# panshengyi/MemVul

Measured on AMD Instinct MI355X. Metric: issue-reports/sec at seq_len=256 (BERT-base issue encoder + 124-anchor memory match), higher is better.
Workload: dtype fp16 + fp8 (MV_F16X8: fp16 MFMA sweep + one OCP-e4m3 MFMA correction sweep per GEMM, fp32 accumulate); 1 GPU; BASELINE.json configs[1]: 1xMI355X-per-rank, bert-base-uncased geometry (12 layers), seq_len=256, batch=256, 124-anchor CWE memory, compute dtype MV_F16X8; seeded random-init weights, synthetic token ids resident in HBM; compute=precise, global_batch=256, seq_len=256, anchors=124, parallelism=dp1 (corpus shards, one all-gather of (score,label) stats), stats_transport=none (one rank)

## Files before the change

### memvul_amd/csrc/gemm_pp.h

```cpp
#pragma once
#include "common.h"
#include <type_traits>
#include "gemm.h"

enum { PP_QK = 1, PP_GELU = 3, PP_RESLN3 = 8 };
constexpr int PP_F = 4;

#define PP_LDS_A 0
#define PP_LDS_B 65536
#define PP_LDS_BIAS 131072
#define PP_LDS_SCR (PP_LDS_BIAS + MV_INTER * 4)
#define PP_LDS_BYTES (PP_LDS_SCR + 8 * 2048)
#define PP_LDS_BIAS_T PP_LDS_BIAS
#define PP_LDS_STATS (PP_LDS_BIAS + 2048)
#define PP_LDS_SCR_RAW (PP_LDS_STATS + 2 * 6144)
#define PP_LDS_RSTD (PP_LDS_SCR_RAW + 8 * 2048)
#define PP_LDS_BYTES_RAW (PP_LDS_RSTD + 2048)

__device__ __forceinline__ uint32_t pack_h2(float a, float b) {
  const half2_t h = {(half_t)a, (half_t)b};
  return __builtin_bit_cast(uint32_t, h);
}

__device__ __forceinline__ void pin_f32x4(float& a, float& b, float& c, float& d) {
#if defined(__HIP_DEVICE_COMPILE__)
  asm("" : "+v"(a), "+v"(b), "+v"(c), "+v"(d));
#endif
}

__device__ __forceinline__ uint32_t f2u(float x) { return __float_as_uint(x); }
__device__ __forceinline__ float u2f(uint32_t x) { return __uint_as_float(x); }
typedef uint32_t u32x2 __attribute__((ext_vector_type(2)));
typedef uint32_t u32x4 __attribute__((ext_vector_type(4)));
typedef int intx4 __attribute__((ext_vector_type(4)));
typedef int intx8 __attribute__((ext_vector_type(8)));

__device__ __forceinline__ void scr_f16x2(uint32_t w0, uint32_t w1, uint32_t w2, uint32_t w3, const u32x2 (&da)[4],
                                          const u32x2 (&db)[4], uint32_t r, u32x4 (&o)[4]) {
#if defined(__HIP_DEVICE_COMPILE__)
  asm volatile(
      "ds_write_b64 %4, %8\n\tds_write_b64 %5, %9\n\tds_write_b64 %6, %10\n\tds_write_b64 %7, %11\n\t"
      "ds_read_b128 %0, %16\n\tds_read_b128 %1, %16 offset:1024\n\t"
      "ds_write_b64 %4, %12\n\tds_write_b64 %5, %13\n\tds_write_b64 %6, %14\n\tds_write_b64 %7, %15\n\t"
      "ds_read_b128 %2, %16\n\tds_read_b128 %3, %16 offset:1024\n\ts_waitcnt lgkmcnt(0)"
      : "=&v"(o[0]), "=&v"(o[1]), "=&v"(o[2]), "=&v"(o[3])
      : "v"(w0), "v"(w1), "v"(w2), "v"(w3), "v"(da[0]), "v"(da[1]), "v"(da[2]), "v"(da[3]), "v"(db[0]), "v"(db[1]),
        "v"(db[2]), "v"(db[3]), "v"(r)
      : "memory");
#endif
}
__device__ __forceinline__ void scr_f8x2(uint32_t w0, uint32_t w1, uint32_t w2, uint32_t w3, const uint32_t (&da)[8],
                                           const uint32_t (&db)[8], uint32_t r, u32x4 (&o)[4]) {
#if defined(__HIP_DEVICE_COMPILE__)
  asm volatile(
      "ds_write_b32 %4, %8\n\tds_write_b32 %5, %9\n\tds_write_b32 %6, %10\n\tds_write_b32 %7, %11\n\t"
      "ds_write_b32 %4, %12 offset:1024\n\tds_write_b32 %5, %13 offset:1024\n\tds_write_b32 %6, %14 offset:1024\n\tds_write_b32 %7, %15 offset:1024\n\t"
      "ds_read_b128 %0, %24\n\tds_read_b128 %1, %24 offset:1024\n\t"
      "ds_write_b32 %4, %16\n\tds_write_b32 %5, %17\n\tds_write_b32 %6, %18\n\tds_write_b32 %7, %19\n\t"
      "ds_write_b32 %4, %20 offset:1024\n\tds_write_b32 %5, %21 offset:1024\n\tds_write_b32 %6, %22 offset:1024\n\tds_write_b32 %7, %23 offset:1024\n\t"
      "ds_read_b128 %2, %24\n\tds_read_b128 %3, %24 offset:1024\n\ts_waitcnt lgkmcnt(0)"
      : "=&v"(o[0]), "=&v"(o[1]), "=&v"(o[2]), "=&v"(o[3])
      : "v"(w0), "v"(w1), "v"(w2), "v"(w3), "v"(da[0]), "v"(da[1]), "v"(da[2]), "v"(da[3]), "v"(da[4]), "v"(da[5]), "v"(da[6]),
        "v"(da[7]), "v"(db[0]), "v"(db[1]), "v"(db[2]), "v"(db[3]), "v"(db[4]), "v"(db[5]), "v"(db[6]), "v"(db[7]), "v"(r)
      : "memory");
#endif
}
__device__ __forceinline__ void scr_f8x1(uint32_t w0, uint32_t w1, uint32_t w2, uint32_t w3, const uint32_t (&da)[8], uint32_t r, u32x4 (&o)[4]) {
#if defined(__HIP_DEVICE_COMPILE__)
  asm volatile(
      "ds_write_b32 %2, %6\n\tds_write_b32 %3, %7\n\tds_write_b32 %4, %8\n\tds_write_b32 %5, %9\n\t"
      "ds_write_b32 %2, %10 offset:1024\n\tds_write_b32 %3, %11 offset:1024\n\tds_write_b32 %4, %12 offset:1024\n\tds_write_b32 %5, %13 offset:1024\n\t"
      "ds_read_b128 %0, %14\n\tds_read_b128 %1, %14 offset:1024\n\ts_waitcnt lgkmcnt(0)"
      : "=&v"(o[0]), "=&v"(o[1])
      : "v"(w0), "v"(w1), "v"(w2), "v"(w3), "v"(da[0]), "v"(da[1]), "v"(da[2]), "v"(da[3]), "v"(da[4]), "v"(da[5]), "v"(da[6]), "v"(da[7]), "v"(r)
      : "memory");
#endif
}
__device__ __forceinline__ void scr_f16x2_t(uint32_t t0, uint32_t t1, const u32x2 (&da)[4], const u32x2 (&db)[4], uint32_t r, u32x4 (&o)[4]) {
#if defined(__HIP_DEVICE_COMPILE__)
  const uint32_t a00 = da[0][0], a01 = da[0][1], a10 = da[1][0], a11 = da[1][1], a20 = da[2][0], a21 = da[2][1], a30 = da[3][0],
                 a31 = da[3][1];
  const uint32_t b00 = db[0][0], b01 = db[0][1], b10 = db[1][0], b11 = db[1][1], b20 = db[2][0], b21 = db[2][1], b30 = db[3][0],
                 b31 = db[3][1];
#define MV_T16(A, LO, HI, OFF)                                                                            \
  "ds_write_b16 " A ", " LO " offset:" #OFF "+0\n\tds_write_b16_d16_hi " A ", " LO " offset:" #OFF "+64\n\t" \
  "ds_write_b16 " A ", " HI " offset:" #OFF "+128\n\tds_write_b16_d16_hi " A ", " HI " offset:" #OFF "+192\n\t"
  asm volatile(
      MV_T16("%4", "%6", "%7", 0) MV_T16("%4", "%8", "%9", 1024) MV_T16("%5", "%10", "%11", 0) MV_T16("%5", "%12", "%13", 1024)
      "ds_read_b128 %0, %22\n\tds_read_b128 %1, %22 offset:1024\n\t"
      MV_T16("%4", "%14", "%15", 0) MV_T16("%4", "%16", "%17", 1024) MV_T16("%5", "%18", "%19", 0) MV_T16("%5", "%20", "%21", 1024)
      "ds_read_b128 %2, %22\n\tds_read_b128 %3, %22 offset:1024\n\ts_waitcnt lgkmcnt(0)"
      : "=&v"(o[0]), "=&v"(o[1]), "=&v"(o[2]), "=&v"(o[3])
      : "v"(t0), "v"(t1), "v"(a00), "v"(a01), "v"(a10), "v"(a11), "v"(a20), "v"(a21), "v"(a30), "v"(a31), "v"(b00), "v"(b01),
        "v"(b10), "v"(b11), "v"(b20), "v"(b21), "v"(b30), "v"(b31), "v"(r)
      : "memory");
#undef MV_T16
#endif
}
__device__ __forceinline__ void scr_f16_rev2(uint32_t wc, const u32x4& a0, const u32x4& a1, const u32x4& b0, const u32x4& b1, uint32_t r0,
                                             uint32_t r1, uint32_t r2, uint32_t r3, u32x2 (&oa)[4], u32x2 (&ob)[4]) {
#if defined(__HIP_DEVICE_COMPILE__)
  asm volatile(
      "ds_write_b128 %8, %9\n\tds_write_b128 %8, %10 offset:1024\n\t"
      "ds_read_b64 %0, %13\n\tds_read_b64 %1, %14\n\tds_read_b64 %2, %15\n\tds_read_b64 %3, %16\n\t"
      "ds_write_b128 %8, %11\n\tds_write_b128 %8, %12 offset:1024\n\t"
      "ds_read_b64 %4, %13\n\tds_read_b64 %5, %14\n\tds_read_b64 %6, %15\n\tds_read_b64 %7, %16\n\ts_waitcnt lgkmcnt(0)"
      : "=&v"(oa[0]), "=&v"(oa[1]), "=&v"(oa[2]), "=&v"(oa[3]), "=&v"(ob[0]), "=&v"(ob[1]), "=&v"(ob[2]), "=&v"(ob[3])
      : "v"(wc), "v"(a0), "v"(a1), "v"(b0), "v"(b1), "v"(r0), "v"(r1), "v"(r2), "v"(r3)
      : "memory");
  __builtin_amdgcn_sched_barrier(0);
#endif
}


__device__ __forceinline__ void lds_read_bgb1(uint32_t addr, float4& bi, float4& ga, float4& be) {
#if defined(__HIP_DEVICE_COMPILE__)
  asm volatile("ds_read_b128 %0, %3\n\tds_read_b128 %1, %3 offset:3072\n\tds_read_b128 %2, %3 offset:6144\n\ts_waitcnt lgkmcnt(0)"
               : "=&v"(bi), "=&v"(ga), "=&v"(be)
               : "v"(addr)
               : "memory");
  __builtin_amdgcn_sched_barrier(0);
#endif
}

__device__ __forceinline__ int sload_i32(const int* p) {
  int v = 0;
#if defined(__HIP_DEVICE_COMPILE__)
  asm volatile("s_load_dword %0, %1, 0x0\n\ts_waitcnt lgkmcnt(0)" : "=s"(v) : "s"(p) : "memory");
#endif
  return v;
}

__device__ __forceinline__ void raster_pp(const GemmArgs& a, int L, int G, int tm_count, int tn_count, int& tile_m, int& tile_n) {
  if (a.raster_mode == 1) {
    const int ngroups = tn_count / a.GN;
    const int w = L / G, r = L - w * G;
    const int b = w / ngroups, g = w - b * ngroups;
    const int p = b * G + r;
    tile_m = p / a.GN;
    tile_n = g * a.GN + (p - tile_m * a.GN);
  } else {
    raster(L, tm_count, tn_count, a.GN, tile_m, tile_n);
  }
}

template <int EPI, int RAW = 0, int X8 = 0>
__global__ __launch_bounds__(512, 2) void gemm_pp_kernel(GemmArgs a) {
  static_assert(EPI == PP_QK || EPI == PP_GELU || EPI == PP_RESLN3, "kernel kinds of the encoder layer");
  static_assert(RAW == (EPI != PP_RESLN3), "PP_QK / PP_GELU consume the raw stream (virtual LayerNorm), PP_RESLN3 produces it");
  constexpr bool IS_RES = (EPI == PP_RESLN3);
  static_assert(X8 == 0 || X8 == 1, "X8 = 1: MV_F16X8 (the fp8 correction sweep)");
  constexpr int WAITN = 2 * PP_F;
  constexpr int LDS_SCR = RAW ? PP_LDS_SCR_RAW : PP_LDS_SCR;
  extern __shared__ __attribute__((aligned(16))) char smem[];
  const int tid = threadIdx.x;
  const int lane = tid & 63;
  const int hi = lane >> 5, l31 = lane & 31;
  const int wave = __builtin_amdgcn_readfirstlane(tid >> 6);
  const int wr = wave >> 2, wc = wave & 3;
  const int K = a.K, nk0 = K >> 6;
  constexpr int nseg = X8 ? 2 : 1;
  auto short_tile = [&](int tm) -> bool { return a.tile_both && sload_i32(a.tile_both + tm) != 0; };
  auto both_terms = [&](int tm, int tn) -> bool {
    if (a.x8_terms == 1) return short_tile(tm);
    if (a.x8_terms != 3) return true;
    const int which = (tn * 256 + a.col0) / MV_HIDDEN;
    return (a.x8_aside_mask >> which) & 1;
  };
  int i_nk8 = X8 ? nk0 : 0;
  size_t i_off8 = 0;
  const int tm_count = a.M >> 8, tn_count = a.N >> 8;
  const int ntiles = tm_count * tn_count;
  const int G = gridDim.x;
  const int bslot = xcd_remap(blockIdx.x, G);

  if constexpr (!RAW) {
    float* lb = (float*)(smem + PP_LDS_BIAS);
    for (int n = tid; n < a.N; n += 512) lb[n] = a.bias ? a.bias[n] : 0.f;
    for (int n = tid; n < MV_HIDDEN; n += 512) {
      lb[MV_HIDDEN + n] = a.lng[n];
      lb[2 * MV_HIDDEN + n] = a.lnb[n];
    }
  }

  uint32_t offA[2], offB[2];
#pragma unroll
  for (int j = 0; j < 2; ++j) {
    const int rho = (2 * wave + j) * 8 + (lane >> 3);
    const int c = (lane & 7) ^ ((rho >> 1) & 7);
    const int rowA = (rho >> 6) * 128 + (rho & 63);
    const int rowB = (rho >> 5) * 64 + (rho & 31);
    offA[j] = (uint32_t)(rowA * K + c * 8) * 2u;
    offB[j] = (uint32_t)(rowB * K + c * 8) * 2u;
  }
  int i_it = 0, i_kt = 0, i_seg = 0;
  const char* iA = (const char*)a.A;
  const char* iW = (const char*)a.W;
  size_t tA = 0, tW = 0;
  auto set_issue_seg = [&]() {
    iA = (i_seg ? (const char*)a.A8 + i_off8 : (const char*)a.A) + tA;
    iW = (i_seg ? (const char*)a.W8 + i_off8 : (const char*)a.W) + tW;
  };
  auto set_issue_tile = [&](int it) {
    const int L = it * G + bslot;
    if (L < ntiles) {
      int tm, tn;
      raster_pp(a, L, G, tm_count, tn_count, tm, tn);
      if constexpr (X8) {
        tA = (size_t)tm * 256 * K * 2;
        tW = (size_t)tn * 256 * K * 2;
        const bool both = both_terms(tm, tn);
        i_nk8 = both ? nk0 : nk0 >> 1;
        i_off8 = both ? 0 : (size_t)K;
      } else {
        iA = (const char*)a.A + (size_t)tm * 256 * K * 2;
        iW = (const char*)a.W + (size_t)tn * 256 * K * 2;
      }
    }
    if constexpr (X8) set_issue_seg();
  };
  set_issue_tile(0);
  auto issue = [&](auto kindc, auto parc) {
    constexpr int kind = decltype(kindc)::value;
    constexpr int par = decltype(parc)::value;
    const char* src;
    char* dst;
    if constexpr (kind < 2) {
      src = iA + (size_t)(kind * 64) * K * 2 + i_kt * 128;
      dst = smem + PP_LDS_A + par * 32768 + kind * 16384 + wave * 2048;
      glds16((const half_t*)(src + offA[0]), dst);
      glds16((const half_t*)(src + offA[1]), dst + 1024);
    } else {
      src = iW + (size_t)((kind - 2) * 32) * K * 2 + i_kt * 128;
      dst = smem + PP_LDS_B + par * 32768 + (kind - 2) * 16384 + wave * 2048;
      glds16((const half_t*)(src + offB[0]), dst);
      glds16((const half_t*)(src + offB[1]), dst + 1024);
    }
    if constexpr (kind == 1) {
      if (++i_kt == ((X8 && i_seg) ? i_nk8 : nk0)) {
        i_kt = 0;
        if constexpr (X8) {
          if (++i_seg == nseg) {
            i_seg = 0;
            set_issue_tile(++i_it);
          } else {
            set_issue_seg();
          }
        } else {
          set_issue_tile(++i_it);
        }
      }
    }
  };
  auto issue_psi = [&](auto psic) {
    constexpr int psi = decltype(psic)::value;
    constexpr int q = psi & 3;
    constexpr int kind = (q == 0) ? 2 : (q == 1) ? 0 : (q == 2) ? 3 : 1;
    issue(std::integral_constant<int, kind>{}, std::integral_constant<int, (psi >> 2) & 1>{});
  };

  const int m16 = lane & 15, q4 = lane >> 4;
  int rdA[2], rdB[2];
#pragma unroll
  for (int kk = 0; kk < 2; ++kk) {
    const int o = m16 * 128 + (((4 * kk + q4) ^ ((m16 >> 1) & 7)) << 4);
    rdA[kk] = PP_LDS_A + wr * 8192 + o;
    rdB[kk] = PP_LDS_B + wc * 4096 + o;
  }
  half8_t Xf[X8 ? 1 : 4][X8 ? 1 : 2], Wx[X8 ? 1 : 2][X8 ? 1 : 2], Wy[X8 ? 1 : 2][X8 ? 1 : 2];
  intx8 Xp[X8 ? 4 : 1], Wxp[X8 ? 2 : 1], Wyp[X8 ? 2 : 1];
  auto ld16 = [&](int off) -> intx4 { return *(const intx4*)(smem + off); };
  auto read_a = [&](int par, int asub) {
#pragma unroll
    for (int t4 = 0; t4 < 4; ++t4) {
      const int o = par * 32768 + asub * 16384 + t4 * 2048;
      if constexpr (X8) {
        Xp[t4] = __builtin_shufflevector(ld16(rdA[0] + o), ld16(rdA[1] + o), 0, 1, 2, 3, 4, 5, 6, 7);
      } else {
#pragma unroll
        for (int kk = 0; kk < 2; ++kk) Xf[t4][kk] = *(const half8_t*)(smem + rdA[kk] + o);
      }
    }
  };
  auto read_b = [&](half8_t (&Wf)[X8 ? 1 : 2][X8 ? 1 : 2], intx8 (&Wp)[X8 ? 2 : 1], int par, int bsub) {
#pragma unroll
    for (int c2 = 0; c2 < 2; ++c2) {
      const int o = par * 32768 + bsub * 16384 + c2 * 2048;
      if constexpr (X8) {
        Wp[c2] = __builtin_shufflevector(ld16(rdB[0] + o), ld16(rdB[1] + o), 0, 1, 2, 3, 4, 5, 6, 7);
      } else {
#pragma unroll
        for (int kk = 0; kk < 2; ++kk) Wf[c2][kk] = *(const half8_t*)(smem + rdB[kk] + o);
      }
    }
  };

  floatx4 acc[8][4];
  auto park_residual = [&](int i, int mw0, int nw0) {
    const int crow = lane >> 2, cchunk = lane & 3;
    bool sp_c = false;
    size_t sp_off = 0;
    if constexpr (X8) {
      if ((i & 1) == 0) {
        const int row0 = mw0 + 32 * i, b = row0 / a.S;
        sp_c = row0 < a.Mreal && b * a.S == row0 && crow < 2;
        sp_off = (size_t)(2 * b + crow) * MV_HIDDEN;
      }
    }
#pragma unroll
    for (int j = 0; j < 2; ++j)
#pragma unroll
      for (int pl = 0; pl < 2; ++pl)
#pragma unroll
        for (int x = 0; x < 2; ++x) {
          const size_t row = (size_t)(mw0 + i * 32 + x * 16 + crow);
          if constexpr (X8) {
            if (pl == 1) {
              float4 t;
              if ((i & 1) == 0 && x == 0 && sp_c) {
                t = *(const float4*)(a.sp_lo_out + sp_off + nw0 + j * 32 + 8 * cchunk);
              } else {
                const float2 u = *(const float2*)(a.out8 + row * (2 * MV_HIDDEN) + nw0 + j * 32 + 8 * cchunk);
                t.x = u.x; t.y = u.y; t.z = 0.f; t.w = 0.f;
              }
              acc[2 * i + 1][2 * j + x][0] = t.x; acc[2 * i + 1][2 * j + x][1] = t.y; acc[2 * i + 1][2 * j + x][2] = t.z; acc[2 * i + 1][2 * j + x][3] = t.w;
              continue;
            }
          }
          const float4 t = *(const float4*)((pl ? a.out16b : a.out16) + row * MV_HIDDEN + nw0 + j * 32 + 8 * cchunk);
          acc[2 * i + pl][2 * j + x][0] = t.x; acc[2 * i + pl][2 * j + x][1] = t.y;
          acc[2 * i + pl][2 * j + x][2] = t.z; acc[2 * i + pl][2 * j + x][3] = t.w;
        }
  };
  auto mma_quadrant = [&](auto asubc, auto bc, auto f8c, const half8_t (&Wf)[X8 ? 1 : 2][X8 ? 1 : 2], const intx8 (&Wp)[X8 ? 2 : 1]) {
    constexpr int asub = decltype(asubc)::value;
    constexpr int b = decltype(bc)::value;
    if constexpr (X8) {
      if constexpr (decltype(f8c)::value) {
#pragma unroll
        for (int c2 = 0; c2 < 2; ++c2)
#pragma unroll
          for (int t4 = 0; t4 < 4; ++t4)
            acc[asub * 4 + t4][b * 2 + c2] = __builtin_amdgcn_mfma_scale_f32_16x16x128_f8f6f4(Wp[c2], Xp[t4], acc[asub * 4 + t4][b * 2 + c2], 0, 0, 0,
                                                                                            a.x8_scale, 0, 0x7f7f7f7f);
      } else {
#pragma unroll
        for (int kk = 0; kk < 2; ++kk)
#pragma unroll
          for (int c2 = 0; c2 < 2; ++c2) {
            const intx4 w4 = kk ? __builtin_shufflevector(Wp[c2], Wp[c2], 4, 5, 6, 7) : __builtin_shufflevector(Wp[c2], Wp[c2], 0, 1, 2, 3);
#pragma unroll
            for (int t4 = 0; t4 < 4; ++t4) {
              const intx4 x4 = kk ? __builtin_shufflevector(Xp[t4], Xp[t4], 4, 5, 6, 7) : __builtin_shufflevector(Xp[t4], Xp[t4], 0, 1, 2, 3);
              acc[asub * 4 + t4][b * 2 + c2] = __builtin_amdgcn_mfma_f32_16x16x32_f16(__builtin_bit_cast(half8_t, w4), __builtin_bit_cast(half8_t, x4),
                                                                                   acc[asub * 4 + t4][b * 2 + c2], 0, 0, 0);
            }
          }
      }
    } else {
#pragma unroll
      for (int kk = 0; kk < 2; ++kk)
#pragma unroll
        for (int c2 = 0; c2 < 2; ++c2)
#pragma unroll
          for (int t4 = 0; t4 < 4; ++t4)
            acc[asub * 4 + t4][b * 2 + c2] = __builtin_amdgcn_mfma_f32_16x16x32_f16(Wf[c2][kk], Xf[t4][kk], acc[asub * 4 + t4][b * 2 + c2], 0, 0, 0);
    }
  };

  auto read_set = [&](auto sc) {
    constexpr int s = decltype(sc)::value & 7;
    constexpr int P = s & 3, par = s >> 2;
    if constexpr (P == 0) { read_a(par, 0); read_b(Wx, Wxp, par, 0); }
    if constexpr (P == 1) read_b(Wy, Wyp, par, 1);
    if constexpr (P == 2) read_a(par, 1);
  };
  auto mma_set = [&](auto sc, auto f8c) {
    constexpr int P = decltype(sc)::value & 3;
    if constexpr (P == 0) mma_quadrant(std::integral_constant<int, 0>{}, std::integral_constant<int, 0>{}, f8c, Wx, Wxp);
    if constexpr (P == 1) mma_quadrant(std::integral_constant<int, 0>{}, std::integral_constant<int, 1>{}, f8c, Wy, Wyp);
    if constexpr (P == 2) mma_quadrant(std::integral_constant<int, 1>{}, std::integral_constant<int, 1>{}, f8c, Wy, Wyp);
    if constexpr (P == 3) mma_quadrant(std::integral_constant<int, 1>{}, std::integral_constant<int, 0>{}, f8c, Wx, Wxp);
  };
  auto interval = [&](auto sc, auto grpc, auto f8c, bool last_of_tile = false) {
    constexpr int s = decltype(sc)::value;
    constexpr int grp = decltype(grpc)::value;
    if constexpr (grp == 0) {
      __builtin_amdgcn_s_setprio(1);
      mma_set(sc, f8c);
      __builtin_amdgcn_s_setprio(0);
      __builtin_amdgcn_sched_barrier(0);
      if (!(s == 7 && last_of_tile)) read_set(std::integral_constant<int, (s + 1) & 7>{});
      issue_psi(std::integral_constant<int, (s + 3 + PP_F) & 7>{});
    } else {
      read_set(sc);
      issue_psi(std::integral_constant<int, (s + 3 + PP_F) & 7>{});
      __builtin_amdgcn_sched_barrier(0);
      mma_set(sc, f8c);
    }
    if constexpr (X8) {
#if defined(__HIP_DEVICE_COMPILE__)
      constexpr int P = s & 3, a0 = (P >= 2) ? 4 : 0, bq = (P == 1 || P == 2) ? 2 : 0;
      asm volatile("" : "+v"(acc[a0][bq]), "+v"(acc[a0 + 1][bq]), "+v"(acc[a0 + 2][bq]), "+v"(acc[a0 + 3][bq]), "+v"(acc[a0][bq + 1]),
                   "+v"(acc[a0 + 1][bq + 1]), "+v"(acc[a0 + 2][bq + 1]), "+v"(acc[a0 + 3][bq + 1]));
#endif
    }
    asm volatile("s_waitcnt vmcnt(%0)" ::"n"(WAITN) : "memory");
    __builtin_amdgcn_sched_barrier(0);
    __builtin_amdgcn_s_barrier();
    __builtin_amdgcn_sched_barrier(0);
  };

  auto issue_stats = [&](int itn, int tm, int tn) {
    if (itn * G + bslot < ntiles && wave < 4) {
#pragma unroll
      for (int pc = 0; pc < 2; ++pc) {
        const int piece = 2 * wave + pc;
        if (piece < 6) {
          const char* src = (const char*)a.lnstats + (size_t)tm * 6144 + piece * 1024 + lane * 16;
          glds16((const half_t*)src, smem + PP_LDS_STATS + (itn & 1) * 6144 + piece * 1024);
        } else if (piece == 6) {
          const char* src = (const char*)a.bias + (size_t)tn * 1024 + lane * 16;
          glds16((const half_t*)src, smem + PP_LDS_BIAS_T + (itn & 1) * 1024);
        }
      }
    }
  };
  if constexpr (RAW) {
    int tm = 0, tn = 0;
    if (bslot < ntiles) raster_pp(a, bslot, G, tm_count, tn_count, tm, tn);
    issue_stats(0, tm, tn);
  }

  issue_psi(std::integral_constant<int, 0>{});
  issue_psi(std::integral_constant<int, 1>{});
  issue_psi(std::integral_constant<int, 2>{});
  issue_psi(std::integral_constant<int, 3>{});
  issue_psi(std::integral_constant<int, 4>{});
  issue_psi(std::integral_constant<int, 5>{});
  issue_psi(std::integral_constant<int, 6>{});
  asm volatile("s_waitcnt vmcnt(%0) lgkmcnt(0)" ::"n"(WAITN) : "memory");
  __builtin_amdgcn_sched_barrier(0);
  __builtin_amdgcn_s_barrier();
  __builtin_amdgcn_sched_barrier(0);

  auto run_tiles = [&](auto grpc) {
  for (int it = 0;; ++it) {
    const int L = it * G + bslot;
    if (L >= ntiles) break;
    int tile_m, tile_n;
    raster_pp(a, L, G, tm_count, tn_count, tile_m, tile_n);
    int next_m = 0, next_n = 0;
    const bool has_next = L + G < ntiles;
    if (has_next) raster_pp(a, L + G, G, tm_count, tn_count, next_m, next_n);
    const int mw = (tile_m << 8) + wr * 128;
    const int nw = (tile_n << 8) + wc * 64;
    bool tile_short = false;
    if constexpr (X8) tile_short = short_tile(tile_m);
    const bool tile_both_terms = X8 && (a.x8_terms == 1 ? tile_short : both_terms(tile_m, tile_n));

    {
      const uint32_t baddr = (uint32_t)(PP_LDS_BIAS + (nw + 4 * q4) * 4);
      const uint32_t scr = (uint32_t)(LDS_SCR + wave * 2048);
      const uint32_t sf = (uint32_t)((m16 >> 2) & 3);
      const uint32_t scr_c = scr + (lane >> 2) * 64 + ((((uint32_t)lane & 3) ^ (((uint32_t)lane >> 4) & 3)) << 4);
      if constexpr (IS_RES) {
        float2 lnst[8];
        float2 lnp[8][3];
#pragma unroll
        for (int tb = 0; tb < 8; ++tb) {
          const float2* pp = (const float2*)(a.lnstats + 6 * (size_t)(mw + tb * 16 + m16));
          lnp[tb][0] = pp[0]; lnp[tb][1] = pp[1]; lnp[tb][2] = pp[2];
        }
        const uint32_t ub = scr + m16 * 64 + (q4 & 1) * 8;
        const uint32_t u00 = ub + ((((uint32_t)(q4 >> 1)) ^ sf) << 4), u01 = ub + (((2u + (uint32_t)(q4 >> 1)) ^ sf) << 4);
        if (it == 0) {
#pragma unroll
          for (int i = 0; i < 4; ++i) park_residual(i, mw, nw);
        }
        if constexpr (X8) {
          const half2_t s8 = {(half_t)(1.0f / (float)(2048 << MV_X8_ACT_SHIFT)), (half_t)(1.0f / (float)(2048 << MV_X8_ACT_SHIFT))};
          const half2_t s11 = {(half_t)(1.0f / 2048.0f), (half_t)(1.0f / 2048.0f)};
#pragma unroll
          for (int i = 0; i < 4; ++i) {
            bool sp_c = false;
            if ((i & 1) == 0) {
              const int row0 = mw + 32 * i, sb0 = row0 / a.S;
              sp_c = row0 < a.Mreal && sb0 * a.S == row0 && (lane >> 2) < 2;
            }
#pragma unroll
            for (int j = 0; j < 2; ++j)
#pragma unroll
              for (int x = 0; x < 2; ++x) {
                floatx4& l = acc[2 * i + 1][2 * j + x];
                const uint32_t w0 = f2u(l[0]), w1 = f2u(l[1]), w2 = f2u(l[2]), w3 = f2u(l[3]);
                half2_t c0 = __builtin_amdgcn_cvt_scalef32_pk_f16_fp8(w0, 1.0f, false) * s8, c1 = __builtin_amdgcn_cvt_scalef32_pk_f16_fp8(w0, 1.0f, true) * s8;
                half2_t c2 = __builtin_amdgcn_cvt_scalef32_pk_f16_fp8(w1, 1.0f, false) * s8, c3 = __builtin_amdgcn_cvt_scalef32_pk_f16_fp8(w1, 1.0f, true) * s8;
                if ((i & 1) == 0 && x == 0 && sp_c) {
                  c0 = __builtin_bit_cast(half2_t, w0) * s11; c1 = __builtin_bit_cast(half2_t, w1) * s11;
                  c2 = __builtin_bit_cast(half2_t, w2) * s11; c3 = __builtin_bit_cast(half2_t, w3) * s11;
                }
                l[0] = u2f(__builtin_bit_cast(uint32_t, c0)); l[1] = u2f(__builtin_bit_cast(uint32_t, c1));
                l[2] = u2f(__builtin_bit_cast(uint32_t, c2)); l[3] = u2f(__builtin_bit_cast(uint32_t, c3));
              }
          }
        }
#pragma unroll
        for (int tb = 0; tb < 8; ++tb) lnst[tb] = ln_from_partials(lnp[tb][0], lnp[tb][1], lnp[tb][2], a.ln_eps);
#pragma unroll
        for (int i = 0; i < 4; ++i) {
#pragma clang fp contract(off)
#pragma unroll
          for (int j = 0; j < 2; ++j) {
            u32x4 p[4];
#pragma unroll
            for (int qq = 0; qq < 4; ++qq)
#pragma unroll
              for (int e = 0; e < 4; ++e) p[qq][e] = f2u(acc[2 * i + (qq >> 1)][2 * j + (qq & 1)][e]);
            u32x2 oh[4], ol[4];
            scr_f16_rev2(scr_c, p[0], p[1], p[2], p[3], u00, u01, u00 + 1024u, u01 + 1024u, oh, ol);
#pragma unroll
            for (int k = 0; k < 4; ++k) {
              const int tbl = k >> 1, cbl = k & 1;
              float4 bi, ga, be;
              lds_read_bgb1(baddr + (2 * j + cbl) * 64, bi, ga, be);
#pragma unroll
              for (int e = 0; e < 4; ++e) {
                const uint32_t wh = oh[k][e >> 1];
                const half2_t h2 = __builtin_bit_cast(half2_t, wh);
                const uint32_t wl = ol[k][e >> 1];
                const half2_t l2 = __builtin_bit_cast(half2_t, wl);
                const float r = (float)h2[e & 1] + (float)l2[e & 1];
                const float t = (r - lnst[2 * i + tbl].x) * lnst[2 * i + tbl].y;
                acc[2 * i + tbl][2 * j + cbl][e] = __builtin_fmaf(t, ((const float*)&ga)[e], ((const float*)&be)[e]) + ((const float*)&bi)[e];
              }
            }
          }
        }
      } else {
#pragma unroll
        for (int tb = 0; tb < 8; ++tb)
#pragma unroll
          for (int cb = 0; cb < 4; ++cb) {
            acc[tb][cb][0] = 0.f; acc[tb][cb][1] = 0.f; acc[tb][cb][2] = 0.f; acc[tb][cb][3] = 0.f;
          }
      }
    }

    if constexpr (decltype(grpc)::value == 0) read_set(std::integral_constant<int, 0>{});
    auto two_ktiles = [&](auto f8c, bool last) {
      interval(std::integral_constant<int, 0>{}, grpc, f8c);
      interval(std::integral_constant<int, 1>{}, grpc, f8c);
      interval(std::integral_constant<int, 2>{}, grpc, f8c);
      interval(std::integral_constant<int, 3>{}, grpc, f8c);
      interval(std::integral_constant<int, 4>{}, grpc, f8c);
      interval(std::integral_constant<int, 5>{}, grpc, f8c);
      interval(std::integral_constant<int, 6>{}, grpc, f8c);
      interval(std::integral_constant<int, 7>{}, grpc, f8c, last);
    };
    for (int kt = 0; kt < nk0; kt += 2) {
      if constexpr (RAW) {
        if (kt == 2) {
          issue_stats(it + 1, next_m, next_n);
          if (wave >= 4) {
            const int row = (wave - 4) * 64 + lane;
            const uint32_t saddr = (uint32_t)(PP_LDS_STATS + (it & 1) * 6144 + row * 24);
            float2 p0, p1, p2;
            asm volatile("ds_read_b64 %0, %3\n\tds_read_b64 %1, %3 offset:8\n\tds_read_b64 %2, %3 offset:16\n\ts_waitcnt lgkmcnt(0)"
                         : "=&v"(p0), "=&v"(p1), "=&v"(p2)
                         : "v"(saddr)
                         : "memory");
            const float rs = ln_from_partials(p0, p1, p2, a.ln_eps).y;
            const uint32_t waddr = (uint32_t)(PP_LDS_RSTD + (it & 1) * 1024 + row * 4);
            asm volatile("ds_write_b32 %0, %1" ::"v"(waddr), "v"(rs) : "memory");
          }
        }
      }
      two_ktiles(std::false_type{}, !X8 && kt + 2 >= nk0);
    }
    if constexpr (X8) {
      const int nk = nk0 + (tile_both_terms ? nk0 : nk0 >> 1);
      for (int kt = nk0; kt < nk; kt += 2) two_ktiles(std::true_type{}, kt + 2 >= nk);
    }

    {
      const uint32_t scr = (uint32_t)(LDS_SCR + wave * 2048);
      const uint32_t sf = (uint32_t)((m16 >> 2) & 3);
      const uint32_t scr_c = scr + (lane >> 2) * 64 + ((((uint32_t)lane & 3) ^ (((uint32_t)lane >> 4) & 3)) << 4);
      const int crow = lane >> 2, cchunk = lane & 3;
      int cls_b[2] = {-1, -1};
      if constexpr (X8) {
        if (a.cls_corr || a.sp_lo_out || a.vlo_sp) {
#pragma unroll
          for (int j = 0; j < 2; ++j) {
            const int row = mw + 64 * j, b = row / a.S;
            if (row < a.Mreal && b * a.S == row) cls_b[j] = b;
          }
        }
        if (a.cls_corr && !tile_both_terms) {
#pragma unroll
          for (int j = 0; j < 2; ++j) {
            if (cls_b[j] >= 0 && m16 < 2) {
              const float* cp = a.cls_corr + (size_t)(2 * cls_b[j] + m16) * a.N + nw + 4 * q4;
              floatx4 c[4];
#pragma unroll
              for (int cb = 0; cb < 4; ++cb) c[cb] = *(const floatx4*)(cp + 16 * cb);
#if defined(__HIP_DEVICE_COMPILE__)
              asm volatile("" : "+v"(c[0]), "+v"(c[1]), "+v"(c[2]), "+v"(c[3]));
#endif
#pragma unroll
              for (int cb = 0; cb < 4; ++cb) {
                acc[4 * j][cb][0] = __builtin_fmaf(c[cb][0], 1.0f / 2048.0f, acc[4 * j][cb][0]);
                acc[4 * j][cb][1] = __builtin_fmaf(c[cb][1], 1.0f / 2048.0f, acc[4 * j][cb][1]);
                acc[4 * j][cb][2] = __builtin_fmaf(c[cb][2], 1.0f / 2048.0f, acc[4 * j][cb][2]);
                acc[4 * j][cb][3] = __builtin_fmaf(c[cb][3], 1.0f / 2048.0f, acc[4 * j][cb][3]);
              }
            }
          }
        }
      }
      if constexpr (IS_RES) {
#pragma unroll
        for (int tb = 0; tb < 8; ++tb) {
          float s1 = 0.f, s2 = 0.f;
#pragma unroll
          for (int cb = 0; cb < 4; ++cb)
#pragma unroll
            for (int e = 0; e < 4; ++e) {
              const float v = acc[tb][cb][e];
              s1 += v;
              s2 = __builtin_fmaf(v, v, s2);
            }
          const auto a1 = __builtin_amdgcn_permlane16_swap(f2u(s1), f2u(s1), false, false);
          const auto a2 = __builtin_amdgcn_permlane16_swap(f2u(s2), f2u(s2), false, false);
          const float h1 = u2f(a1[0]) + u2f(a1[1]), h2 = u2f(a2[0]) + u2f(a2[1]);
          const auto t1 = __builtin_amdgcn_permlane32_swap(f2u(h1), f2u(h1), false, false);
          const auto t2 = __builtin_amdgcn_permlane32_swap(f2u(h2), f2u(h2), false, false);
          float2 st;
          st.x = u2f(t1[0]) + u2f(t1[1]);
          st.y = u2f(t2[0]) + u2f(t2[1]);
          const uint32_t waddr = scr + (uint32_t)(tb * 16 + m16) * 8;
          asm volatile("ds_write_b64 %0, %1" ::"v"(waddr), "v"(st) : "memory");
        }
        asm volatile("s_waitcnt lgkmcnt(0)" ::: "memory");
        __builtin_amdgcn_sched_barrier(0);
        __builtin_amdgcn_s_barrier();
        __builtin_amdgcn_sched_barrier(0);
        if (wc == 0) {
#pragma unroll
          for (int ii = 0; ii < 2; ++ii) {
            const int row = (2 * hi + ii) * 32 + l31;
            const uint32_t raddr = (uint32_t)(LDS_SCR + wr * 4 * 2048) + (uint32_t)row * 8;
            float2 q0, q1, q2, q3;
            asm volatile("ds_read_b64 %0, %4\n\tds_read_b64 %1, %4 offset:2048\n\tds_read_b64 %2, %4 offset:4096\n\t"
                         "ds_read_b64 %3, %4 offset:6144\n\ts_waitcnt lgkmcnt(0)"
                         : "=&v"(q0), "=&v"(q1), "=&v"(q2), "=&v"(q3)
                         : "v"(raddr)
                         : "memory");
            float2 st;
            st.x = ((q0.x + q1.x) + q2.x) + q3.x;
            st.y = ((q0.y + q1.y) + q2.y) + q3.y;
            *(float2*)(a.lnpart + ((size_t)(mw + row) * 3 + tile_n) * 2) = st;
          }
        }
        __builtin_amdgcn_sched_barrier(0);
        __builtin_amdgcn_s_barrier();
        __builtin_amdgcn_sched_barrier(0);
      }
      {
        const uint32_t ub = scr + m16 * 64 + (q4 & 1) * 8;
        const uint32_t u00 = ub + ((((uint32_t)(q4 >> 1)) ^ sf) << 4), u01 = ub + (((2u + (uint32_t)(q4 >> 1)) ^ sf) << 4);
        const uint32_t ub8 = scr + m16 * 64 + q4 * 4;
        half_t* obase;
        size_t rstride;
        size_t istride;
        size_t jstride;
        bool live = true;
        bool vtile = false;
        ptrdiff_t lo_delta = 0;
        const uint32_t tb0 = scr + q4 * 256 + (m16 & 7) * 2;
        const uint32_t tt0 = tb0 + ((((uint32_t)(m16 >> 3)) ^ (uint32_t)q4) << 4), tt1 = tb0 + (((2u + (uint32_t)(m16 >> 3)) ^ (uint32_t)q4) << 4);
        if constexpr (EPI == PP_GELU || IS_RES) {
          obase = a.out16 + (size_t)(mw + crow) * a.N + nw + 8 * cchunk;
          rstride = a.N; istride = (size_t)32 * a.N; jstride = 32;
        } else {
          const int colg = nw + a.col0;
          const int which = colg >= 2 * MV_HIDDEN ? 2 : (colg >= MV_HIDDEN ? 1 : 0);
          const int head = (colg - which * MV_HIDDEN) >> 6;
          vtile = which == 2;
          if (vtile) {
            obase = a.vt + ((size_t)head * MV_HEAD_DIM + crow) * a.S + 8 * cchunk;
            rstride = a.S; istride = 0; jstride = (size_t)32 * a.S;
            if (a.vt_lo) lo_delta = a.vt_lo - a.vt;
          } else {
            obase = (which ? a.k : a.q) + (size_t)head * a.S * MV_HEAD_DIM + (size_t)crow * MV_HEAD_DIM + 8 * cchunk;
            rstride = MV_HEAD_DIM; istride = 0; jstride = 32;
            if (a.vt_lo) lo_delta = which ? a.k_lo - a.k : a.q_lo - a.q;
          }
        }
        float4 rbv[4];
        float rrs[8];
        if constexpr (RAW) {
          const uint32_t baddr = (uint32_t)(PP_LDS_BIAS_T + (it & 1) * 1024 + (wc * 64 + 4 * q4) * 4);
          const uint32_t saddr = (uint32_t)(PP_LDS_RSTD + (it & 1) * 1024 + (wr * 128 + m16) * 4);
          asm volatile(
              "ds_read_b128 %0, %12\n\tds_read_b128 %1, %12 offset:64\n\tds_read_b128 %2, %12 offset:128\n\t"
              "ds_read_b128 %3, %12 offset:192\n\t"
              "ds_read_b32 %4, %13\n\tds_read_b32 %5, %13 offset:64\n\tds_read_b32 %6, %13 offset:128\n\t"
              "ds_read_b32 %7, %13 offset:192\n\tds_read_b32 %8, %13 offset:256\n\tds_read_b32 %9, %13 offset:320\n\t"
              "ds_read_b32 %10, %13 offset:384\n\tds_read_b32 %11, %13 offset:448\n\ts_waitcnt lgkmcnt(0)"
              : "=&v"(rbv[0]), "=&v"(rbv[1]), "=&v"(rbv[2]), "=&v"(rbv[3]), "=&v"(rrs[0]), "=&v"(rrs[1]), "=&v"(rrs[2]), "=&v"(rrs[3]),
                "=&v"(rrs[4]), "=&v"(rrs[5]), "=&v"(rrs[6]), "=&v"(rrs[7])
              : "v"(baddr), "v"(saddr)
              : "memory");
          __builtin_amdgcn_sched_barrier(0);
        }
        (void)ub8;
#pragma unroll
        for (int i = 0; i < 4; ++i) {
          const int mb = mw + i * 32;
          half_t* ob = obase + i * istride;
          if constexpr (EPI == PP_QK) {
            live = mb < a.Mreal;
            const int b = mb / a.S, s0 = mb - b * a.S;
            if (!vtile) ob = obase + ((size_t)b * MV_HEADS * a.S + s0) * MV_HEAD_DIM;
            else ob = obase + (size_t)b * MV_HEADS * MV_HEAD_DIM * a.S + s0;
          }
          u32x2 d[2][4];
          u32x4 o[4];
#pragma unroll
          for (int j = 0; j < 2; ++j)
#pragma unroll
            for (int k = 0; k < 4; ++k) {
              const int tb = 2 * i + (k >> 1), cb = 2 * j + (k & 1);
              float v0 = acc[tb][cb][0], v1 = acc[tb][cb][1], v2 = acc[tb][cb][2], v3 = acc[tb][cb][3];
              if constexpr (RAW) {
                v0 = __builtin_fmaf(rrs[tb], v0, rbv[cb].x); v1 = __builtin_fmaf(rrs[tb], v1, rbv[cb].y);
                v2 = __builtin_fmaf(rrs[tb], v2, rbv[cb].z); v3 = __builtin_fmaf(rrs[tb], v3, rbv[cb].w);
              }
              if constexpr (EPI == PP_GELU) {
                float2_t a01, a23;
                a01.x = v0; a01.y = v1; a23.x = v2; a23.y = v3;
                a01 = gelu_erf2(a01);
                a23 = gelu_erf2(a23);
                v0 = a01.x; v1 = a01.y; v2 = a23.x; v3 = a23.y;
                if constexpr (X8) {
                  acc[tb][cb][0] = v0; acc[tb][cb][1] = v1; acc[tb][cb][2] = v2; acc[tb][cb][3] = v3;
                }
              }
              pin_f32x4(v0, v1, v2, v3);
              d[j][k][0] = pack_h2(v0, v1);
              d[j][k][1] = pack_h2(v2, v3);
            }
          if (EPI == PP_QK && vtile) scr_f16x2_t(tt0, tt1, d[0], d[1], scr_c, o);
          else scr_f16x2(u00, u01, u00 + 1024u, u01 + 1024u, d[0], d[1], scr_c, o);
          if (live) {
#pragma unroll
            for (int j = 0; j < 2; ++j) {
              half_t* op = ob + j * jstride;
              *(u32x4*)op = o[2 * j];
              *(u32x4*)(op + 16 * rstride) = o[2 * j + 1];
            }
          }
          if constexpr (EPI == PP_QK && X8) {
            if (a.vlo_sp && vtile && (i & 1) == 0 && cls_b[i >> 1] >= 0 && m16 < 2) {
              const int head = (nw + a.col0 - 2 * MV_HIDDEN) >> 6;
              half_t* vp = a.vlo_sp + ((size_t)(cls_b[i >> 1] * MV_HEADS + head) * MV_HEAD_DIM + 4 * q4) * 2 + m16;
#pragma unroll
              for (int cb = 0; cb < 4; ++cb) {
                float vv[4] = {__builtin_fmaf(rrs[2 * i], acc[2 * i][cb][0], rbv[cb].x), __builtin_fmaf(rrs[2 * i], acc[2 * i][cb][1], rbv[cb].y),
                               __builtin_fmaf(rrs[2 * i], acc[2 * i][cb][2], rbv[cb].z), __builtin_fmaf(rrs[2 * i], acc[2 * i][cb][3], rbv[cb].w)};
                pin_f32x4(vv[0], vv[1], vv[2], vv[3]);
#pragma unroll
                for (int e = 0; e < 4; ++e) vp[(16 * cb + e) * 2] = (half_t)((vv[e] - (float)(half_t)vv[e]) * 2048.0f);
              }
            }
            if (a.vt_lo) {
#pragma unroll
              for (int j = 0; j < 2; ++j)
#pragma unroll
                for (int k = 0; k < 4; ++k) {
                  const int tb = 2 * i + (k >> 1), cb = 2 * j + (k & 1);
                  float v0 = __builtin_fmaf(rrs[tb], acc[tb][cb][0], rbv[cb].x), v1 = __builtin_fmaf(rrs[tb], acc[tb][cb][1], rbv[cb].y);
                  float v2 = __builtin_fmaf(rrs[tb], acc[tb][cb][2], rbv[cb].z), v3 = __builtin_fmaf(rrs[tb], acc[tb][cb][3], rbv[cb].w);
                  pin_f32x4(v0, v1, v2, v3);
                  d[j][k][0] = pack_h2(v0 - (float)(half_t)v0, v1 - (float)(half_t)v1);
                  d[j][k][1] = pack_h2(v2 - (float)(half_t)v2, v3 - (float)(half_t)v3);
                }
              if (vtile) scr_f16x2_t(tt0, tt1, d[0], d[1], scr_c, o);
              else scr_f16x2(u00, u01, u00 + 1024u, u01 + 1024u, d[0], d[1], scr_c, o);
              if (live) {
                half_t* ol = ob + lo_delta;
#pragma unroll
                for (int j = 0; j < 2; ++j) {
                  half_t* op = ol + j * jstride;
                  *(u32x4*)op = o[2 * j];
                  *(u32x4*)(op + 16 * rstride) = o[2 * j + 1];
                }
              }
            }
          }
          if constexpr (IS_RES && !X8) {
#pragma unroll
            for (int j = 0; j < 2; ++j)
#pragma unroll
              for (int k = 0; k < 4; ++k) {
                const int tb = 2 * i + (k >> 1), cb = 2 * j + (k & 1);
                const float v0 = acc[tb][cb][0], v1 = acc[tb][cb][1], v2 = acc[tb][cb][2], v3 = acc[tb][cb][3];
                d[j][k][0] = pack_h2(v0 - (float)(half_t)v0, v1 - (float)(half_t)v1);
                d[j][k][1] = pack_h2(v2 - (float)(half_t)v2, v3 - (float)(half_t)v3);
              }
            scr_f16x2(u00, u01, u00 + 1024u, u01 + 1024u, d[0], d[1], scr_c, o);
            half_t* ol = ob + (a.out16b - a.out16);
#pragma unroll
            for (int j = 0; j < 2; ++j) {
              half_t* op = ol + j * jstride;
              *(u32x4*)op = o[2 * j];
              *(u32x4*)(op + 16 * rstride) = o[2 * j + 1];
            }
          }
          if constexpr (X8 && (IS_RES || EPI == PP_GELU)) {
            uint32_t dl[8], dh[8];
            float vmax8 = 0.f;
            const uint32_t w8 = ub8 + (sf << 4);
            uint8_t* o8 = a.out8 + (size_t)(mb + crow) * (2 * a.N) + nw + 16 * cchunk;
            bool hi_only = false;
            if constexpr (X8) hi_only = a.out8_hi_only && !tile_short;
            if (a.sp_lo_out && (i & 1) == 0 && cls_b[i >> 1] >= 0 && m16 < 2) {
              half_t* sp = a.sp_lo_out + (size_t)(2 * cls_b[i >> 1] + m16) * a.N + nw + 4 * q4;
#pragma unroll
              for (int cb = 0; cb < 4; ++cb) {
                half4_t l;
#pragma unroll
                for (int e = 0; e < 4; ++e) {
                  const float v = acc[2 * i][cb][e];
                  l[e] = (half_t)((v - (float)(half_t)v) * 2048.0f);
                }
                *(half4_t*)(sp + 16 * cb) = l;
              }
            }
#pragma unroll
            for (int tbl = 0; tbl < 2; ++tbl)
#pragma unroll
              for (int j = 0; j < 2; ++j)
#pragma unroll
                for (int cbl = 0; cbl < 2; ++cbl) {
                  const int tb = 2 * i + tbl, cb = 2 * j + cbl, u = 4 * tbl + 2 * j + cbl;
                  if (hi_only) {
                    dh[u] = x8_hi4_in_range(acc[tb][cb][0], acc[tb][cb][1], acc[tb][cb][2], acc[tb][cb][3]);
                  } else if constexpr (EPI == PP_GELU) {
                    const uint32_t p01 = d[j][2 * tbl + cbl][0], p23 = d[j][2 * tbl + cbl][1];
                    x8_planes4_in_range_packed(acc[tb][cb][0], acc[tb][cb][1], acc[tb][cb][2], acc[tb][cb][3], p01, p23, dh[u], dl[u]);
                  } else {
                    x8_planes4_in_range(acc[tb][cb][0], acc[tb][cb][1], acc[tb][cb][2], acc[tb][cb][3], dh[u], dl[u]);
                  }
                  vmax8 = x8_absmax4(vmax8, acc[tb][cb][0], acc[tb][cb][1], acc[tb][cb][2], acc[tb][cb][3]);
                }
            if (x8_any_out_of_range(vmax8)) {
              int n = 0;
#pragma unroll
              for (int tbl = 0; tbl < 2; ++tbl)
#pragma unroll
                for (int j = 0; j < 2; ++j)
#pragma unroll
                  for (int cbl = 0; cbl < 2; ++cbl) {
                    const int tb = 2 * i + tbl, cb = 2 * j + cbl;
                    x8_planes4(acc[tb][cb][0], acc[tb][cb][1], acc[tb][cb][2], acc[tb][cb][3], dh[4 * tbl + 2 * j + cbl], dl[4 * tbl + 2 * j + cbl]);
                    n += x8_count4(acc[tb][cb][0], acc[tb][cb][1], acc[tb][cb][2], acc[tb][cb][3]);
                  }
              x8_sat_add(a.x8_sat, n);
            }
            if (hi_only) {
              scr_f8x1(w8, w8 ^ 16u, w8 ^ 32u, w8 ^ 48u, dh, scr_c, o);
              *(u32x4*)(o8 + a.N) = o[0];
              *(u32x4*)(o8 + a.N + (size_t)16 * (2 * a.N)) = o[1];
            } else {
              scr_f8x2(w8, w8 ^ 16u, w8 ^ 32u, w8 ^ 48u, dl, dh, scr_c, o);
              *(u32x4*)o8 = o[0];
              *(u32x4*)(o8 + (size_t)16 * (2 * a.N)) = o[1];
              *(u32x4*)(o8 + a.N) = o[2];
              *(u32x4*)(o8 + a.N + (size_t)16 * (2 * a.N)) = o[3];
            }
          }
          if constexpr (IS_RES) {
            if (has_next) park_residual(i, (next_m << 8) + wr * 128, (next_n << 8) + wc * 64);
          }
        }
      }
    }
  }
  };
  if (wr == 0) run_tiles(std::integral_constant<int, 0>{});
  else run_tiles(std::integral_constant<int, 1>{});

  asm volatile("s_waitcnt vmcnt(0)" ::: "memory");
}
```

Measured before the change: 14820 issue-reports/s.

## Prefetch CLS correction rows into LDS asynchronously and defer prologue for residual GEMMs

The CLS-row fp8 correction values used to be read from global memory with direct vector loads in the epilogue. They are now fetched with an async global-to-LDS copy issued early in the K loop (at kt==2) into the per-wave scratch, and the epilogue reads them back with ds_read_b128. Separately, for residual GEMMs the initial operand prefetch prologue is moved to run after the residual tiles are parked on the first tile. The intent is to hide global latency in the epilogue and reorder the initial loads, at the cost of scratch-LDS reuse hazards and more complex lane-index arithmetic.

Result: no change. 14830 issue-reports/s (median of 3 runs) (+0.0%).

```diff
diff --git a/memvul_amd/csrc/gemm_pp.h b/memvul_amd/csrc/gemm_pp.h
--- a/memvul_amd/csrc/gemm_pp.h
+++ b/memvul_amd/csrc/gemm_pp.h
@@ -426,23 +426,34 @@
       }
     }
   };
+  auto issue_row_piece = [&](int b0, int b1, int nw) {
+    uint32_t l = 0;
+#if defined(__HIP_DEVICE_COMPILE__)
+    asm volatile("v_mbcnt_lo_u32_b32 %0, -1, 0\n\tv_mbcnt_hi_u32_b32 %0, -1, %0" : "=v"(l));
+#endif
+    const uint32_t base0 = (uint32_t)(2 * (b0 < 0 ? 0 : b0) * a.N + nw) * 4u, base1 = (uint32_t)(2 * (b1 < 0 ? 0 : b1) * a.N + nw) * 4u;
+    const uint32_t off = ((l >> 5) ? base1 : base0) + ((l >> 4) & 1) * (uint32_t)(a.N * 4) + 16u * (l & 15);
+    glds16((const half_t*)((const char*)a.cls_corr + off), smem + LDS_SCR + wave * 2048);
+  };
   if constexpr (RAW) {
     int tm = 0, tn = 0;
     if (bslot < ntiles) raster_pp(a, bslot, G, tm_count, tn_count, tm, tn);
     issue_stats(0, tm, tn);
   }
-
-  issue_psi(std::integral_constant<int, 0>{});
-  issue_psi(std::integral_constant<int, 1>{});
-  issue_psi(std::integral_constant<int, 2>{});
-  issue_psi(std::integral_constant<int, 3>{});
-  issue_psi(std::integral_constant<int, 4>{});
-  issue_psi(std::integral_constant<int, 5>{});
-  issue_psi(std::integral_constant<int, 6>{});
-  asm volatile("s_waitcnt vmcnt(%0) lgkmcnt(0)" ::"n"(WAITN) : "memory");
-  __builtin_amdgcn_sched_barrier(0);
-  __builtin_amdgcn_s_barrier();
-  __builtin_amdgcn_sched_barrier(0);
+  auto prologue = [&]() {
+    issue_psi(std::integral_constant<int, 0>{});
+    issue_psi(std::integral_constant<int, 1>{});
+    issue_psi(std::integral_constant<int, 2>{});
+    issue_psi(std::integral_constant<int, 3>{});
+    issue_psi(std::integral_constant<int, 4>{});
+    issue_psi(std::integral_constant<int, 5>{});
+    issue_psi(std::integral_constant<int, 6>{});
+    asm volatile("s_waitcnt vmcnt(%0) lgkmcnt(0)" ::"n"(WAITN) : "memory");
+    __builtin_amdgcn_sched_barrier(0);
+    __builtin_amdgcn_s_barrier();
+    __builtin_amdgcn_sched_barrier(0);
+  };
+  if constexpr (!IS_RES) prologue();
 
   auto run_tiles = [&](auto grpc) {
   for (int it = 0;; ++it) {
@@ -458,6 +469,18 @@
     bool tile_short = false;
     if constexpr (X8) tile_short = short_tile(tile_m);
     const bool tile_both_terms = X8 && (a.x8_terms == 1 ? tile_short : both_terms(tile_m, tile_n));
+    int piece_b[2] = {-1, -1};
+    bool row_piece = false;
+    if constexpr (X8) {
+      if (a.cls_corr && !tile_both_terms) {
+#pragma unroll
+        for (int j = 0; j < 2; ++j) {
+          const int row = mw + 64 * j, b = row / a.S;
+          if (row < a.Mreal && b * a.S == row) piece_b[j] = b;
+        }
+        row_piece = piece_b[0] >= 0 || piece_b[1] >= 0;
+      }
+    }
 
     {
       const uint32_t baddr = (uint32_t)(PP_LDS_BIAS + (nw + 4 * q4) * 4);
@@ -477,6 +500,8 @@
         if (it == 0) {
 #pragma unroll
           for (int i = 0; i < 4; ++i) park_residual(i, mw, nw);
+          __builtin_amdgcn_sched_barrier(0);
+          prologue();
         }
         if constexpr (X8) {
           const half2_t s8 = {(half_t)(1.0f / (float)(2048 << MV_X8_ACT_SHIFT)), (half_t)(1.0f / (float)(2048 << MV_X8_ACT_SHIFT))};
@@ -576,6 +601,9 @@
           }
         }
       }
+      if constexpr (X8) {
+        if (kt == 2 && row_piece) issue_row_piece(piece_b[0], piece_b[1], nw);
+      }
       two_ktiles(std::false_type{}, !X8 && kt + 2 >= nk0);
     }
     if constexpr (X8) {
@@ -597,16 +625,22 @@
             if (row < a.Mreal && b * a.S == row) cls_b[j] = b;
           }
         }
-        if (a.cls_corr && !tile_both_terms) {
+        if (row_piece) {
+          uint32_t l = 0;
+#if defined(__HIP_DEVICE_COMPILE__)
+          asm volatile("v_mbcnt_lo_u32_b32 %0, -1, 0\n\tv_mbcnt_hi_u32_b32 %0, -1, %0" : "=v"(l));
+#endif
 #pragma unroll
           for (int j = 0; j < 2; ++j) {
-            if (cls_b[j] >= 0 && m16 < 2) {
-              const float* cp = a.cls_corr + (size_t)(2 * cls_b[j] + m16) * a.N + nw + 4 * q4;
-              floatx4 c[4];
-#pragma unroll
-              for (int cb = 0; cb < 4; ++cb) c[cb] = *(const floatx4*)(cp + 16 * cb);
-#if defined(__HIP_DEVICE_COMPILE__)
-              asm volatile("" : "+v"(c[0]), "+v"(c[1]), "+v"(c[2]), "+v"(c[3]));
+            if (cls_b[j] >= 0 && (l & 15) < 2) {
+              floatx4 c[4] = {};
+#if defined(__HIP_DEVICE_COMPILE__)
+              const uint32_t caddr = scr + 512u * j + 256u * (l & 15) + 16u * (l >> 4);
+              asm volatile("ds_read_b128 %0, %4\n\tds_read_b128 %1, %4 offset:64\n\tds_read_b128 %2, %4 offset:128\n\tds_read_b128 %3, %4 offset:192\n\t"
+                           "s_waitcnt lgkmcnt(0)"
+                           : "=&v"(c[0]), "=&v"(c[1]), "=&v"(c[2]), "=&v"(c[3])
+                           : "v"(caddr)
+                           : "memory");
 #endif
 #pragma unroll
               for (int cb = 0; cb < 4; ++cb) {
```
